# DH-Ng/TacEx

Hardware: AMD Instinct MI355X
Metric: tactile_frames_per_sec (higher is better)
Workload: dtype f32; 1 GPU; 1024 envs x 2 GelSight Mini per GPU = 2048 frames/step/GPU, Taxim RGB 320x240 + FOTS markers (99); BASELINE configs[2] (C3); envs_per_gpu=1024, sensors_per_env=2, markers=True, sensors=group, gather=obs32 u8 (9551872 B/rank, N=1: no collective), arch=gfx950:sramecc+:xnack-

## Files before the change

tacex_amd/csrc/fots_kernels.hip:

```cpp
#include <hip/hip_runtime.h>
#include <math.h>

#include <algorithm>
#include <stdint.h>

#include "tacex_hip.h"
#include "tacex_internal.h"

namespace tacex {

typedef float v4f __attribute__((ext_vector_type(4)));

__global__ __launch_bounds__(1024) void fots_reduce_kernel(const float* __restrict__ z,
                                                          const uint8_t* __restrict__ mask,
                                                          FotsReduce* __restrict__ out, int H, int W) {
  const int e = blockIdx.x;
  const int npix = H * W;
  const float* zz = z + (size_t)e * npix;
  const uint8_t* mm = mask + (size_t)e * npix;
  float zmax = -INFINITY;
  int cnt = 0, sr = 0, sc = 0;
  const int n4 = npix >> 2;
  for (int i = threadIdx.x; i < n4; i += blockDim.x) {
    v4f v = reinterpret_cast<const v4f*>(zz)[i];
    uchar4 m = reinterpret_cast<const uchar4*>(mm)[i];
    zmax = fmaxf(zmax, fmaxf(fmaxf(v[0], v[1]), fmaxf(v[2], v[3])));
    const int p = i << 2;
    const int row = p / W, col = p - row * W;
    const int c = (m.x != 0) + (m.y != 0) + (m.z != 0) + (m.w != 0);
    cnt += c;
    sr += c * row;
    sc += (m.x != 0) * col + (m.y != 0) * (col + 1) + (m.z != 0) * (col + 2) + (m.w != 0) * (col + 3);
  }
#pragma unroll
  for (int o = 32; o > 0; o >>= 1) {
    zmax = fmaxf(zmax, __shfl_xor(zmax, o, 64));
    cnt += __shfl_xor(cnt, o, 64);
    sr += __shfl_xor(sr, o, 64);
    sc += __shfl_xor(sc, o, 64);
  }
  __shared__ float s_z[16];
  __shared__ int s_c[16], s_r[16], s_k[16];
  const int wid = threadIdx.x >> 6;
  if ((threadIdx.x & 63) == 0) { s_z[wid] = zmax; s_c[wid] = cnt; s_r[wid] = sr; s_k[wid] = sc; }
  __syncthreads();
  if (threadIdx.x == 0) {
    const int nw = blockDim.x >> 6;
    for (int w = 1; w < nw; ++w) { zmax = fmaxf(zmax, s_z[w]); cnt += s_c[w]; sr += s_r[w]; sc += s_k[w]; }
    out[e].zmax = zmax; out[e].count = cnt; out[e].sum_row = sr; out[e].sum_col = sc;
  }
}

__global__ __launch_bounds__(64) void fots_combine_kernel(const FotsReduce* __restrict__ part, int n, FotsReduce* __restrict__ out) {
  const int e = blockIdx.x;
  const FotsReduce* p = part + (size_t)e * n;
  float zmax = -INFINITY;
  int cnt = 0, sr = 0, sc = 0;
  for (int i = threadIdx.x; i < n; i += 64) {
    const FotsReduce r = p[i];
    zmax = fmaxf(zmax, r.zmax); cnt += r.count; sr += r.sum_row; sc += r.sum_col;
  }
#pragma unroll
  for (int o = 32; o > 0; o >>= 1) {
    zmax = fmaxf(zmax, __shfl_xor(zmax, o, 64));
    cnt += __shfl_xor(cnt, o, 64);
    sr += __shfl_xor(sr, o, 64);
    sc += __shfl_xor(sc, o, 64);
  }
  if (threadIdx.x == 0) { out[e].zmax = zmax; out[e].count = cnt; out[e].sum_row = sr; out[e].sum_col = sc; }
}

struct FotsArgs {
  const float* z; const uint8_t* mask; const float* indent; const float* theta;
  float* traj; float* markers; const FotsReduce* red;
  const int* mx; const int* my;
  int B, H, W, nrow, ncol;
  int compact;
  double lamb0, lamb1, lamb2;
  float mm2pix, shear_max, theta_max_rad_f;
};

__device__ __forceinline__ int centre_px(float t, float mm2pix, float half) {
  float prod = t * mm2pix;
  asm volatile("" : "+v"(prod));
  return (int)(prod + half);
}

__global__ __launch_bounds__(128) void fots_marker_kernel(FotsArgs a) {
  const int e = blockIdx.x;
  const int M = a.nrow * a.ncol;
  const int tid = threadIdx.x;
  __shared__ float s_gmax;
  __shared__ int s_ncontact;
  __shared__ int s_cy[128], s_cx[128];
  __shared__ double s_ch[128];
  __shared__ int s_flag[128];

  float g = -INFINITY;
  for (int i = tid; i < a.B; i += blockDim.x) g = fmaxf(g, a.red[i].zmax);
#pragma unroll
  for (int o = 32; o > 0; o >>= 1) g = fmaxf(g, __shfl_xor(g, o, 64));
  __shared__ float s_g2[2];
  if ((tid & 63) == 0) s_g2[tid >> 6] = g;
  __syncthreads();
  if (tid == 0) s_gmax = fmaxf(s_g2[0], s_g2[1]);
  __syncthreads();
  const float gmax = s_gmax;
  const FotsReduce red = a.red[e];
  const size_t fo = (size_t)e * a.H * a.W;
  float* out_init = a.markers + (size_t)e * 2 * M * 2;
  float* out_cur = out_init + (size_t)M * 2;
  float* tr = a.traj + (size_t)e * 8;
  const bool in_contact = a.indent[e] > 0.0f;

  const bool active = tid < M;
  int j = 0, i = 0, px = 0, py = 0;
  if (active) { j = tid / a.ncol; i = tid - j * a.ncol; px = a.mx[tid]; py = a.my[tid]; }
  if (active) { out_init[tid * 2 + 0] = (float)px; out_init[tid * 2 + 1] = (float)py; }

  if (!in_contact) {
    if (active) { out_cur[tid * 2 + 0] = (float)px; out_cur[tid * 2 + 1] = (float)py; }
    if (tid == 0) { tr[0] = 0.0f; tr[7] = 0.0f; }
    return;
  }

  bool hit = false;
  float hval = 0.0f;
  if (active && py >= 0 && py < a.H && px >= 0 && px < a.W) {
    const size_t pi = a.compact ? (size_t)e * M + tid : fo + (size_t)py * a.W + px;
    if (a.mask[pi] == 1) {
      hit = true;
      const float dz = gmax - a.z[pi];
      const float dmin = gmax - red.zmax;
      hval = (dz - dmin) / 10.0f;
    }
  }
  s_flag[tid] = hit ? 1 : 0;
  __syncthreads();
  if (hit) {
    const int key = i * a.nrow + j;
    int rank = 0;
    for (int m2 = 0; m2 < M; ++m2) {
      if (s_flag[m2]) {
        const int j2 = m2 / a.ncol, i2 = m2 - j2 * a.ncol;
        rank += (i2 * a.nrow + j2) < key;
      }
    }
    s_cy[rank] = py; s_cx[rank] = px; s_ch[rank] = (double)hval;
  }
  if (tid == 0) {
    int n = 0;
    for (int m2 = 0; m2 < M; ++m2) n += s_flag[m2];
    s_ncontact = n;
  }
  __syncthreads();
  const int nc = s_ncontact;

  float t0x, t0y, t0t, tlx, tly, tlt;
  int tlen;
  {
    const float mean_r = (float)((double)red.sum_row / (double)red.count);
    const float mean_c = (float)((double)red.sum_col / (double)red.count);
    const float cy = (mean_r - (float)(a.H / 2.0)) / a.mm2pix;
    const float cx = (mean_c - (float)(a.W / 2.0)) / a.mm2pix;
    const float th = a.theta[e];
    tlen = (int)tr[0];
    if (tlen == 0) { t0x = cx; t0y = cy; t0t = th; } else { t0x = tr[1]; t0y = tr[2]; t0t = tr[3]; }
    tlx = cx; tly = cy; tlt = th;
    tlen += 1;
  }
  __syncthreads();
  if (tid == 0) {
    tr[0] = (float)tlen; tr[1] = t0x; tr[2] = t0y; tr[3] = t0t; tr[4] = tlx; tr[5] = tly; tr[6] = tlt;
    tr[7] = (float)nc;
  }
  if (!active) return;

  if (nc == 0) {
    out_cur[tid * 2 + 0] = (float)px; out_cur[tid * 2 + 1] = (float)py;
    return;
  }

  double dx = 0.0, dy = 0.0;
  for (int c = 0; c < nc; ++c) {
    const double ox = (double)(px - s_cx[c]), oy = (double)(py - s_cy[c]);
    const double gg = exp(-a.lamb0 * (ox * ox + oy * oy));
    dx += s_ch[c] * ox * gg;
    dy += s_ch[c] * oy * gg;
  }
  double nx = (double)px + dx, ny = (double)py + dy;

  if (tlen >= 2) {
    const float half_w = (float)(a.W / 2.0), half_h = (float)(a.H / 2.0);
    const int scx = centre_px(t0x, a.mm2pix, half_w);
    const int scy = centre_px(t0y, a.mm2pix, half_h);
    int shx = (int)((tlx - t0x) * a.mm2pix);
    int shy = (int)((tly - t0y) * a.mm2pix);
    const int smax = (int)a.shear_max;
    shx = shx < -smax ? -smax : (shx > smax ? smax : shx);
    shy = shy < -smax ? -smax : (shy > smax ? smax : shy);
    {
      const double ox = (double)(px - scx), oy = (double)(py - scy);
      const double gg = exp(-a.lamb1 * (ox * ox + oy * oy));
      nx += (double)shx * gg;
      ny += (double)shy * gg;
    }
    float theta = tlt - t0t;
    theta = fminf(fmaxf(theta, -a.theta_max_rad_f), a.theta_max_rad_f);
    const int tcx = centre_px(tlx, a.mm2pix, half_w);
    const int tcy = centre_px(tly, a.mm2pix, half_h);
    const double c1 = (double)cosf(theta - 1.0f);
    const double s1 = (double)sinf(theta);
    const double ox = (double)(px - tcx), oy = (double)(py - tcy);
    const double gg = exp(-a.lamb2 * (ox * ox + oy * oy));
    nx += (ox * c1 - oy * s1) * gg;
    ny += (ox * s1 + oy * c1) * gg;
  }
  out_cur[tid * 2 + 0] = (float)nx;
  out_cur[tid * 2 + 1] = (float)ny;
}


struct MarkerImgArgs {
  const float* markers;
  const uint8_t* patches;
  const float* rgb;
  uint8_t* img;
  uint8_t* overlay;
  int B, M, H, W, SR, S, patch_w;
  int band_rows, nbands;
};
constexpr int kMkPad = 12, kMkPatch = 12;

__global__ __launch_bounds__(256) void fots_marker_image_kernel(MarkerImgArgs a) {
  extern __shared__ __attribute__((aligned(16))) uint8_t canvas[];
  const int e = blockIdx.x / a.nbands, band = blockIdx.x - e * a.nbands;
  const int CW = a.W + 2 * kMkPad, CH = a.H + 2 * kMkPad;
  const int y0 = band * a.band_rows, y1 = min(CH, y0 + a.band_rows);
  const int tid = threadIdx.x;
  for (int i = tid * 4; i < (y1 - y0) * CW; i += 256 * 4) *reinterpret_cast<uint32_t*>(canvas + i) = 0xffffffffu;
  __syncthreads();
  const float* cur = a.markers + ((size_t)e * 2 + 1) * a.M * 2;
  for (int m = 0; m < a.M; ++m) {
    const double u = ((double)cur[m * 2 + 0] + 0.5) + 12.0, v = ((double)cur[m * 2 + 1] + 0.5) + 12.0;
    const double fu = floor(u), fv = floor(v);
    const int pu = (int)floor((u - fu) * a.SR), pv = (int)floor((v - fv) * a.SR);
    const int cu = (int)fu - 6, cv = (int)fv - 6;
    const bool ok = u == u && v == v && fabs(u) < 1e9 && fabs(v) < 1e9 && cu >= 0 && cu < CW - 12 && cv >= 0 && cv < CH - 12;
    if (ok && cv + kMkPatch > y0 && cv < y1 && tid < kMkPatch * kMkPatch) {
      const int dy = tid / kMkPatch, dx = tid - dy * kMkPatch, yy = cv + dy;
      if (yy >= y0 && yy < y1)
        canvas[(yy - y0) * CW + cu + dx] =
            a.patches[((((size_t)pu * a.SR + pv) * a.S + a.patch_w) * kMkPatch + dy) * kMkPatch + dx];
    }
    __syncthreads();
  }
  const int r0 = max(y0, kMkPad), r1 = min(y1, a.H + kMkPad);
  for (int i = tid; i < (r1 - r0) * a.W; i += 256) {
    const int ry = i / a.W, x = i - ry * a.W;
    const uint8_t mv = canvas[(r0 + ry - y0) * CW + kMkPad + x];
    const size_t p = ((size_t)e * a.H + (r0 + ry - kMkPad)) * a.W + x;
    if (a.img) a.img[p] = mv;
    if (a.overlay) {
      const double f = (double)mv / 255.0;
#pragma unroll
      for (int ch = 0; ch < 3; ++ch) a.overlay[p * 3 + ch] = (uint8_t)(int)((double)(a.rgb[p * 3 + ch] * 255.0f) * f);
    }
  }
}

}

using namespace tacex;

struct tacex_fots_ctx {
  int device = 0;
  int H = 0, W = 0, nrow = 0, ncol = 0;
  int* mx_dev = nullptr;
  int* my_dev = nullptr;
  double lamb[3];
  float mm2pix, shear_max, theta_max_deg;
};

extern "C" {

int tacex_fots_create(int device_id, const tacex_fots_params* p, tacex_fots_ctx** out) {
  if (!p || !out || !p->marker_x || !p->marker_y) { set_error("tacex_fots_create: null argument"); return 2; }
  const int M = p->num_markers_row * p->num_markers_col;
  if (M <= 0 || M > 128) { set_error("tacex_fots_create: %d markers unsupported (1..128)", M); return 2; }
  if (p->width % 4 != 0) { set_error("tacex_fots_create: image width %d must be a multiple of 4", p->width); return 2; }
  hipError_t e = hipSetDevice(device_id);
  if (e != hipSuccess) return fail_hip(e, "hipSetDevice");
  auto* c = new tacex_fots_ctx();
  c->device = device_id; c->H = p->height; c->W = p->width; c->nrow = p->num_markers_row; c->ncol = p->num_markers_col;
  for (int k = 0; k < 3; ++k) c->lamb[k] = p->lamb[k];
  c->mm2pix = p->mm2pix; c->shear_max = p->shear_max; c->theta_max_deg = p->theta_max_deg;
  if ((e = hipMalloc((void**)&c->mx_dev, M * sizeof(int))) != hipSuccess ||
      (e = hipMalloc((void**)&c->my_dev, M * sizeof(int))) != hipSuccess ||
      (e = hipMemcpy(c->mx_dev, p->marker_x, M * sizeof(int), hipMemcpyHostToDevice)) != hipSuccess ||
      (e = hipMemcpy(c->my_dev, p->marker_y, M * sizeof(int), hipMemcpyHostToDevice)) != hipSuccess) {
    tacex_fots_destroy(c);
    return fail_hip(e, "tacex_fots_create: table upload");
  }
  *out = c;
  return 0;
}

void tacex_fots_destroy(tacex_fots_ctx* c) {
  if (!c) return;
  (void)hipSetDevice(c->device);
  if (c->mx_dev) (void)hipFree(c->mx_dev);
  if (c->my_dev) (void)hipFree(c->my_dev);
  delete c;
}

size_t tacex_fots_state_bytes(int num_envs) { return num_envs > 0 ? (size_t)num_envs * 8 * sizeof(float) : 0; }
size_t tacex_fots_workspace_bytes(int num_envs) { return num_envs > 0 ? (size_t)num_envs * sizeof(FotsReduce) : 0; }

static int fots_markers_impl(tacex_fots_ctx* c, const float* z, const uint8_t* mask, const float* indent, const float* theta,
                             float* traj_state, float* markers, void* ws, const FotsReduce* part, int npart, int B, void* stream, int compact = 0);

int tacex_fots_markers(tacex_fots_ctx* c, const float* z, const uint8_t* mask, const float* indent,
                       const float* theta, float* traj_state, float* markers, void* ws, int B, void* stream) {
  if (!c || !z || !mask || !indent || !theta || !traj_state || !markers || !ws) {
    set_error("tacex_fots_markers: null argument");
    return 2;
  }
  if (B <= 0) return 0;
  return fots_markers_impl(c, z, mask, indent, theta, traj_state, markers, ws, nullptr, 0, B, stream);
}

int tacex_fots_markers_partials(tacex_fots_ctx* c, const float* z, const uint8_t* mask, const float* indent,
                                const float* theta, float* traj_state, float* markers, void* ws, const void* partials,
                                int partials_per_env, int B, void* stream) {
  if (!c || !z || !mask || !indent || !theta || !traj_state || !markers || !ws || !partials || partials_per_env < 1) {
    set_error("tacex_fots_markers_partials: null argument");
    return 2;
  }
  if (B <= 0) return 0;
  return fots_markers_impl(c, z, mask, indent, theta, traj_state, markers, ws, static_cast<const FotsReduce*>(partials),
                           partials_per_env, B, stream);
}

int tacex_fots_markers_compact(tacex_fots_ctx* c, const float* z_pix, const uint8_t* mask_pix, const float* indent,
                               const float* theta, float* traj_state, float* markers, void* ws, const void* partials,
                               int partials_per_env, int B, void* stream) {
  if (!c || !z_pix || !mask_pix || !indent || !theta || !traj_state || !markers || !ws || !partials || partials_per_env < 1) {
    set_error("tacex_fots_markers_compact: null argument");
    return 2;
  }
  if (B <= 0) return 0;
  return fots_markers_impl(c, z_pix, mask_pix, indent, theta, traj_state, markers, ws, static_cast<const FotsReduce*>(partials),
                           partials_per_env, B, stream, 1);
}

static int fots_markers_impl(tacex_fots_ctx* c, const float* z, const uint8_t* mask, const float* indent, const float* theta,
                             float* traj_state, float* markers, void* ws, const FotsReduce* part, int npart, int B, void* stream, int compact) {
  hipStream_t st = (hipStream_t)stream;
  FotsReduce* red = static_cast<FotsReduce*>(ws);
  if (part) hipLaunchKernelGGL(fots_combine_kernel, dim3(B), dim3(64), 0, st, part, npart, red);
  else hipLaunchKernelGGL(fots_reduce_kernel, dim3(B), dim3(1024), 0, st, z, mask, red, c->H, c->W);
  FotsArgs a{};
  a.compact = compact;
  a.z = z; a.mask = mask; a.indent = indent; a.theta = theta; a.traj = traj_state; a.markers = markers; a.red = red;
  a.mx = c->mx_dev; a.my = c->my_dev; a.B = B; a.H = c->H; a.W = c->W; a.nrow = c->nrow; a.ncol = c->ncol;
  a.lamb0 = c->lamb[0]; a.lamb1 = c->lamb[1]; a.lamb2 = c->lamb[2];
  a.mm2pix = c->mm2pix; a.shear_max = c->shear_max;
  a.theta_max_rad_f = (float)(c->theta_max_deg / 180.0 * 3.14159265358979323846);
  hipLaunchKernelGGL(fots_marker_kernel, dim3(B), dim3(128), 0, st, a);
  hipError_t e = hipGetLastError();
  if (e != hipSuccess) return fail_hip(e, "fots kernels");
  return 0;
}

int tacex_fots_marker_image(const float* markers, const uint8_t* patches, int super_res, int size_slots, int patch_w,
                            const float* rgb, uint8_t* img, uint8_t* overlay, int B, int M, int H, int W, void* stream) {
  if (!markers || !patches || (!img && !overlay)) { set_error("tacex_fots_marker_image: null argument"); return 2; }
  if (overlay && !rgb) { set_error("tacex_fots_marker_image: the overlay needs the RGB frame"); return 2; }
  if (super_res < 1 || size_slots < 1 || patch_w < 0 || patch_w >= size_slots) {
    set_error("tacex_fots_marker_image: patch table index %d outside [0, %d)", patch_w, size_slots);
    return 2;
  }
  if (W % 4 != 0 || H <= 0 || W <= 0 || M < 0) { set_error("tacex_fots_marker_image: need W %% 4 == 0, H > 0"); return 2; }
  if (B <= 0) return 0;
  MarkerImgArgs a{};
  a.markers = markers; a.patches = patches; a.rgb = rgb; a.img = img; a.overlay = overlay;
  a.B = B; a.M = M; a.H = H; a.W = W; a.SR = super_res; a.S = size_slots; a.patch_w = patch_w;
  const int CW = W + 2 * kMkPad, CH = H + 2 * kMkPad;
  const size_t budget = 96 * 1024;
  a.band_rows = (int)std::min<size_t>((size_t)CH, budget / CW);
  if (a.band_rows < 2 * kMkPatch) { set_error("tacex_fots_marker_image: image too wide (%d)", W); return 2; }
  a.nbands = (CH + a.band_rows - 1) / a.band_rows;
  const size_t lds = (size_t)a.band_rows * CW;
  auto kern = fots_marker_image_kernel;
  static size_t granted[64] = {};
  if (hipError_t e = ensure_dynamic_lds(reinterpret_cast<const void*>(kern), lds, granted); e != hipSuccess)
    return fail_hip(e, "hipFuncSetAttribute(fots_marker_image_kernel)");
  hipLaunchKernelGGL(kern, dim3(B * a.nbands), dim3(256), lds, (hipStream_t)stream, a);
  hipError_t e = hipGetLastError();
  return e == hipSuccess ? 0 : fail_hip(e, "fots_marker_image_kernel");
}

}
```

tacex_amd/csrc/taxim_device.h:

```cpp
#pragma once
#include <hip/hip_runtime.h>
#include <stdint.h>

#include <type_traits>

#include "tacex_internal.h"
#include "wave_ops.h"

namespace tacex {

typedef float v2f __attribute__((ext_vector_type(2)));
typedef float v4f __attribute__((ext_vector_type(4)));

template <int I, int N, typename F>
__device__ __forceinline__ void static_for(F&& f) {
  if constexpr (I < N) {
    f(std::integral_constant<int, I>{});
    static_for<I + 1, N>(f);
  }
}

__device__ __forceinline__ float fmin_raw(float a, float b) {
  float r;
  asm("v_min_f32 %0, %1, %2" : "=v"(r) : "v"(a), "v"(b));
// ... 83 lines not shown
__device__ __forceinline__ void shade_bins(const ShadeArgs& a, float ztop, float zbot, float zlef, float zrig, int& im,
                                           int& id) {
  const float dzdx = (ztop - zbot) * a.gsy;
  const float dzdy = (zlef - zrig) * a.gsx;
  const float t = __builtin_amdgcn_sqrtf(fmaf(dzdx, dzdx, dzdy * dzdy));
  const float mag = atan_pos(t);
  const float dir = t != 0.0f ? atan2_fast(dzdx, dzdy) : 0.0f;
  im = min((int)(mag * a.inv_x_binr), a.nb - 1);
  id = min((int)((dir + 3.14159274101257324f) * a.inv_y_binr), a.nb - 1);
}

__device__ __forceinline__ int shade_dir_bin(const ShadeArgs& a, float dzdx, float dzdy, float t2) {
  const float dir = !(t2 < 1.17549435e-38f) ? atan2_fast(dzdx, dzdy) : 0.0f;
  return min((int)((dir + 3.14159274101257324f) * a.inv_y_binr), a.nb - 1);
}
__device__ __forceinline__ int shade_mag_bin(const ShadeArgs& a, float t2) {
  return min((int)(atan_pos(__builtin_amdgcn_sqrtf(t2)) * a.inv_x_binr), a.nb - 1);
}

__device__ __forceinline__ void shade_poly(const ShadeArgs& a, int im, int id, float X, float Y, float out[3]) {
  const v4f* __restrict__ pc =
      reinterpret_cast<const v4f*>(reinterpret_cast<const char*>(a.poly) + (unsigned)(im * a.nb + id) * 96u);
  const v4f c0 = pc[0], c1 = pc[1], c2 = pc[2], c3 = pc[3], c4 = pc[4];
  const float f0 = X * X, f1 = Y * Y, f2 = X * Y;
  out[0] = fmaf(f0, c0.x, fmaf(f1, c0.y, fmaf(f2, c0.z, fmaf(X, c0.w, fmaf(Y, c1.x, c1.y)))));
  out[1] = fmaf(f0, c1.z, fmaf(f1, c1.w, fmaf(f2, c2.x, fmaf(X, c2.y, fmaf(Y, c2.z, c2.w)))));
  out[2] = fmaf(f0, c3.x, fmaf(f1, c3.y, fmaf(f2, c3.z, fmaf(X, c3.w, fmaf(Y, c4.x, c4.y)))));
}

__device__ __forceinline__ void shade_pixel_core(const ShadeArgs& a, float ztop, float zbot, float zlef, float zrig,
                                                 int x, int y, float out[3], int& im_out, int& id_out) {
  const unsigned p = (unsigned)y * (unsigned)a.W + (unsigned)x;
  int im, id;
  shade_bins(a, ztop, zbot, zlef, zrig, im, id);
  float c[3];
  shade_poly(a, im, id, a.fx[(unsigned)x], a.fy[(unsigned)y], c);
  const float* __restrict__ bg = reinterpret_cast<const float*>(reinterpret_cast<const char*>(a.bg) + p * 12u);
  out[0] = __builtin_amdgcn_fmed3f(c[0] + bg[0], 0.0f, 1.0f);
  out[1] = __builtin_amdgcn_fmed3f(c[1] + bg[1], 0.0f, 1.0f);
  out[2] = __builtin_amdgcn_fmed3f(c[2] + bg[2], 0.0f, 1.0f);
  im_out = im;
  id_out = id;
}

__device__ __forceinline__ void shade_pixel_rgb(const ShadeArgs& a, float ztop, float zbot, float zlef, float zrig, int x,
                                                int y, float out[3]) {
  int im, id;
  shade_pixel_core(a, ztop, zbot, zlef, zrig, x, y, out, im, id);
}

__device__ __forceinline__ void shade_strip4_rgb(const ShadeArgs& a, const float zn[4][4], int x, int y, float out[12]) {
  const unsigned p = (unsigned)y * (unsigned)a.W + (unsigned)x;
  const v4f X4 = *reinterpret_cast<const v4f*>(a.fx + (unsigned)x);
  const float Y = a.fy[(unsigned)y];
  const v4f* __restrict__ bgp = reinterpret_cast<const v4f*>(reinterpret_cast<const char*>(a.bg) + p * 12u);
  const v4f b0 = bgp[0], b1 = bgp[1], b2 = bgp[2];
  const float bg[12] = {b0.x, b0.y, b0.z, b0.w, b1.x, b1.y, b1.z, b1.w, b2.x, b2.y, b2.z, b2.w};
#pragma unroll
  for (int i = 0; i < 4; ++i) {
    int im, id;
    shade_bins(a, zn[i][0], zn[i][1], zn[i][2], zn[i][3], im, id);
    float c[3];
    shade_poly(a, im, id, X4[i], Y, c);
#pragma unroll
    for (int ch = 0; ch < 3; ++ch) out[3 * i + ch] = __builtin_amdgcn_fmed3f(c[ch] + bg[3 * i + ch], 0.0f, 1.0f);
  }
}

__device__ __forceinline__ void shade_pixel(const ShadeArgs& a, float ztop, float zbot, float zlef, float zrig, int x,
                                            int y, int b) {
  float c[3];
  int im, id;
  shade_pixel_core(a, ztop, zbot, zlef, zrig, x, y, c, im, id);
  const size_t p = (size_t)y * a.W + x;
  float* __restrict__ o = a.rgb + ((size_t)b * a.H * a.W + p) * 3;
  o[0] = c[0]; o[1] = c[1]; o[2] = c[2];
  if (a.idx_out) {
    uint8_t* io = a.idx_out + ((size_t)b * a.H * a.W + p) * 2;
    io[0] = (uint8_t)im;
    io[1] = (uint8_t)id;
  }
}

template <bool U8, typename G>
__device__ __forceinline__ void obs_finish_cell(void* __restrict__ obs_v, const ObsTables& T, G&& gather) {
  const int oh = T.oh, ow = T.ow;
  const int cell = blockIdx.x * blockDim.x + threadIdx.x;
  if (cell >= oh * ow) return;
  const int b = blockIdx.y;
  const int oy = cell / ow, ox = cell - oy * ow;
  float a0 = 0.0f, a1 = 0.0f, a2 = 0.0f;
  gather(b, oy, ox, a0, a1, a2);
  const float nrm = T.xsum[ox] * T.ysum[oy];
  const size_t oi = ((size_t)b * (oh * ow) + cell) * 3;
  if constexpr (U8) {
    uint8_t* o = static_cast<uint8_t*>(obs_v) + oi;
    o[0] = (uint8_t)(a0 / nrm * 255.0f + 0.5f); o[1] = (uint8_t)(a1 / nrm * 255.0f + 0.5f); o[2] = (uint8_t)(a2 / nrm * 255.0f + 0.5f);
  } else {
    float* o = static_cast<float*>(obs_v) + oi;
    o[0] = a0 / nrm; o[1] = a1 / nrm; o[2] = a2 / nrm;
  }
}
template <typename K, typename... A>
inline hipError_t launch_obs_finish(bool u8, K kern_u8, K kern_f32, const ObsTables& t, int B, hipStream_t st, A... args) {
  const dim3 grid((t.oh * t.ow + 255) / 256, B);
  hipLaunchKernelGGL(u8 ? kern_u8 : kern_f32, grid, dim3(256), 0, st, args...);
  return hipGetLastError();
}

}
```

tacex_amd/csrc/taxim_stream.hip:

```cpp
#include <hip/hip_runtime.h>
#include <stdint.h>
#include <stdlib.h>

#include <type_traits>
#include <vector>

#include "tacex_internal.h"
#include "taxim_device.h"

namespace tacex {

constexpr int kStreamPx = 3;
constexpr int kStreamWaves = 4;
constexpr int kStreamObsActive = 3;

struct StreamArgs {
  const float* zin;
  const float* hm;
  const float* gel;
  const float* shift_a;
  const float* shift_b;
  const float* pdepth;
  const float* taps[kStreamMaxLevels];
  ShadeArgs sh;
// ... 902 lines not shown
    if (do_obs) {
      obs_flush(OA[0], cur_o0);
      obs_flush(OA[1], cur_o0 + 1);
      obs_flush(OA[2], cur_o0 + 2);
    }
  }
  if (do_fots) {
    f_zmax = wave_scan_max_lane63(f_zmax);
    int f_sc = 0;
#pragma unroll
    for (int i = 0; i < PX; ++i) f_sc += f_cpx[i] * xg[i];
    f_sc = wave_scan_add_lane63(f_sc);
    if (lane == 63) {
      FotsReduce r;
      r.zmax = f_zmax; r.count = f_cnt; r.sum_row = f_sr; r.sum_col = f_sc;
      a.fots_part[(size_t)frame * a.fots_stride + rem] = r;
    }
    if (rem == 0) {
      FotsReduce id;
      id.zmax = -INFINITY; id.count = 0; id.sum_row = 0; id.sum_col = 0;
      for (int s2 = per_frame + lane; s2 < a.fots_stride; s2 += 64) a.fots_part[(size_t)frame * a.fots_stride + s2] = id;
    }
  }
}

__global__ __launch_bounds__(256) void stream_flat_image_kernel(ShadeArgs sh, float* __restrict__ out) {
  const int x = blockIdx.x * blockDim.x + threadIdx.x, y = blockIdx.y;
  if (x >= sh.W) return;
  const int code = shade_dir_bin(sh, 0.0f, 0.0f, 0.0f);
  const StreamRec r = stream_rec_load(sh.poly + (size_t)code * 24);
  float p0, p1, p2;
  stream_poly(sh.fx[x], sh.fy[y], r, p0, p1, p2);
  const float* bg = sh.bg + ((size_t)y * sh.W + x) * 3;
  float* o = out + ((size_t)y * sh.W + x) * 3;
  o[0] = __builtin_amdgcn_fmed3f(p0 + bg[0], 0.0f, 1.0f);
  o[1] = __builtin_amdgcn_fmed3f(p1 + bg[1], 0.0f, 1.0f);
  o[2] = __builtin_amdgcn_fmed3f(p2 + bg[2], 0.0f, 1.0f);
}

__global__ __launch_bounds__(1024) void stream_order_kernel(const int* __restrict__ rows_ext, int n_items, int per_frame, int nseg,
                                                            int seg_rows, int H, int reach, int* __restrict__ order) {
  constexpr int kKeys = 1024;
  __shared__ int hist[kKeys], start[kKeys];
  for (int k = threadIdx.x; k < kKeys; k += blockDim.x) hist[k] = 0;
  __syncthreads();
  auto key_of = [&](int item) {
    const int frame = item / per_frame, seg = (item - frame * per_frame) % nseg;
    const int r0 = seg * seg_rows, r1 = min(H, r0 + seg_rows);
    const int lo = rows_ext[4 * frame], hi = rows_ext[4 * frame + 1];
    if ((r0 - reach > hi) || (r1 + reach < lo)) return 0;
    const int pad = 4;
    const int c = min(r1 - 1, hi + pad) - max(r0, lo - pad) + 1;
    return min(kKeys - 1, 1 + max(c, 0));
  };
  for (int i = threadIdx.x; i < n_items; i += blockDim.x) atomicAdd(&hist[key_of(i)], 1);
  __syncthreads();
  if (threadIdx.x == 0) {
    int acc = 0;
    for (int k = min(kKeys - 1, seg_rows + 9); k >= 0; --k) { start[k] = acc; acc += hist[k]; }
  }
  __syncthreads();
  for (int i = threadIdx.x; i < n_items; i += blockDim.x) order[atomicAdd(&start[key_of(i)], 1)] = i;
}

template <bool U8>
__global__ __launch_bounds__(256) void obs_finish_stream_kernel(const float* __restrict__ part, void* __restrict__ obs_v, ObsTables T,
                                                               const int* __restrict__ strip_q0, const int* __restrict__ strip_nq,
                                                               const int* __restrict__ seg_oa, const int* __restrict__ seg_ob,
                                                               int nstrips, int nseg, int nrows, int ncols) {
  obs_finish_cell<U8>(obs_v, T, [&](int b, int oy, int ox, float& a0, float& a1, float& a2) {
    for (int s = 0; s < nstrips; ++s) {
      const int qi = ox - strip_q0[s];
      if (qi < 0 || qi >= strip_nq[s]) continue;
      for (int g = 0; g < nseg; ++g) {
        if (oy < seg_oa[g] || oy > seg_ob[g]) continue;
        const size_t blk = ((size_t)b * nstrips + s) * nseg + g;
        const float* pp = part + blk * ((size_t)nrows * ncols * 3) + ((size_t)(oy - seg_oa[g]) * ncols + qi) * 3;
        a0 += pp[0]; a1 += pp[1]; a2 += pp[2];
      }
    }
  });
}

template <int ROLE, bool ST, int... KS>
constexpr StreamCfg<ROLE, KS...> stream_cfg(FusedSet<ST, KS...>) { return {}; }

template <typename C>
static bool stream_geometry_t(int W, int* nstrips, int* strip_w) {
  int ns = (W + C::VW - 1) / C::VW;
  int sw = (((W + ns - 1) / ns) + 3) & ~3;
  if (sw > C::VW) { ++ns; sw = (((W + ns - 1) / ns) + 3) & ~3; }
  *nstrips = ns;
  *strip_w = sw;
  return sw <= C::VW;
}

static bool stream_split() {
  static const int v = getenv("TACEX_STREAM_SPLIT") ? atoi(getenv("TACEX_STREAM_SPLIT")) : 0;
  return v != 0;
}

bool stream_supported(int n_fused, int k0, int H, int W) {
  static const int en = getenv("TACEX_TAIL_STREAM") ? atoi(getenv("TACEX_TAIL_STREAM")) : 1;
  return en != 0 && with_stream_set(n_fused, k0, false, [](auto) { return true; }) && H >= 16 && W >= 16 && W % 4 == 0;
}

bool stream_geometry(int n_fused, int k0, int W, int* nstrips, int* strip_w, int* lv_nstrips, int* lv_strip_w) {
  return with_stream_set(n_fused, k0, false, [&](auto s) {
    if (stream_split())
      return stream_geometry_t<StreamCfg<kStreamShade>>(W, nstrips, strip_w) &&
             stream_geometry_t<decltype(stream_cfg<kStreamLevels>(s))>(W, lv_nstrips, lv_strip_w);
    const bool ok = stream_geometry_t<decltype(stream_cfg<kStreamFused>(s))>(W, nstrips, strip_w);
    *lv_nstrips = *nstrips; *lv_strip_w = *strip_w;
    return ok;
  });
}

int stream_segments(int B, int nstrips, int H, int warm, int per_simd) {
  static const int forced = getenv("TACEX_STREAM_SEGS") ? atoi(getenv("TACEX_STREAM_SEGS")) : 0;
  int nseg = forced > 0 ? forced : (1024 * per_simd + B * nstrips - 1) / (B * nstrips);
  if (nseg < 1) nseg = 1;
  if (nseg > kStreamMaxSeg) nseg = kStreamMaxSeg;
  const int min_rows = forced > 0 ? 24 : (3 * warm > 24 ? 3 * warm : 24);
  while (nseg > 1 && (H / nseg < min_rows || H - (nseg - 1) * ((H + nseg - 1) / nseg) < 4)) --nseg;
  return nseg;
}
int stream_waves_per_simd(int n_fused, int k0) {
  return with_stream_set(n_fused, k0, 2, [](auto s) { return decltype(stream_cfg<kStreamFused>(s))::min_waves(); });
}
static int stream_sum_r(int n_fused, int k0) {
  return with_stream_set(n_fused, k0, 0, [](auto s) { return decltype(stream_cfg<kStreamFused>(s))::sum_r(); });
}
int stream_warm_rows(int n_fused, int k0, bool levels_kernel) {
  const int sum_r = stream_sum_r(n_fused, k0);
  if (!stream_split()) return 2 * sum_r + 2;
  return levels_kernel ? 2 * sum_r : 2;
}

template <bool GZ, int ROLE, int... KS>
static hipError_t launch_stream_k(const StreamArgs& a, hipStream_t st) {
  using C = StreamCfg<ROLE, KS...>;
  const int waves = a.B * a.nstrips * a.nseg;
  const int nwg = (waves + kStreamWaves - 1) / kStreamWaves;
  const dim3 grid(nwg);
  static const size_t lds_pad = getenv("TACEX_STREAM_LDS_PAD") ? (size_t)atoi(getenv("TACEX_STREAM_LDS_PAD")) : 0;
  const size_t lds = C::lds_bytes() + lds_pad;
  auto kern = taxim_stream_kernel<GZ, ROLE, C::min_waves(), KS...>;
  static size_t granted[64] = {};
  if (hipError_t e = ensure_dynamic_lds(reinterpret_cast<const void*>(kern), lds, granted); e != hipSuccess) return e;
  hipLaunchKernelGGL(kern, grid, dim3(64 * kStreamWaves), lds, st, a);
  return hipGetLastError();
}

template <int ROLE, bool ST, int... KS>
static hipError_t launch_stream(FusedSet<ST, KS...>, const StreamArgs& a, bool gel_zero, hipStream_t st) {
  return gel_zero ? launch_stream_k<true, ROLE, KS...>(a, st) : launch_stream_k<false, ROLE, KS...>(a, st);
}

hipError_t run_stream_flat_image(const ShadeParams* sp, int H, int W, hipStream_t st) {
  if (!sp->flat_rgb_dev) return hipErrorInvalidValue;
  hipLaunchKernelGGL(stream_flat_image_kernel, dim3((W + 255) / 256, H), dim3(256), 0, st, make_shade_args(*sp, 1, H, W), sp->flat_rgb_dev);
  return hipGetLastError();
}

static bool stream_sorted() {
  static const int sorted = getenv("TACEX_STREAM_ORDER") ? atoi(getenv("TACEX_STREAM_ORDER")) : 1;
// ... 7 lines not shown
  return hipGetLastError();
}

hipError_t run_stream_order(const LevelDesc* lv, int n_levels, int n_fused, const StreamPlan& plan, int B, int H, const int* rows_ext, int ext_grow,
                            int* order_buf, hipStream_t st, bool* launched) {
  *launched = false;
  if (stream_split() || !stream_sorted() || !order_buf || !lv[0].gel_zero || !rows_ext) return hipSuccess;
  const hipError_t e = launch_stream_order(stream_sum_r(n_fused, lv[n_levels - n_fused].kw), rows_ext, ext_grow, B, plan.nstrips, plan.nseg,
                                           plan.seg_rows, H, order_buf, st);
  *launched = e == hipSuccess;
  return e;
}

bool stream_tail_range_aware(const LevelDesc* lv) {
#ifdef TACEX_STREAM_HM_ALWAYS
  return false;
#else
  return lv[0].gel_zero;
#endif
}

hipError_t run_stream_tail(const LevelDesc* lv, int n_levels, int n_fused, const float* zin, const float* hm, const float* gel,
                           const float* sa, const float* sb, const float* pd, const ShadeParams* sp, float* rgb, float* z_last,
                           int B, int H, int W, float contact_scale, const StreamPlan& plan, float* obs_part,
                           FotsReduce* fots_part, int fots_stride, float* pix_z, uint8_t* pix_m, hipStream_t st,
                           const int* rows_ext, int ext_grow, int* order_buf, bool order_done) {
  const bool sorted = stream_sorted();
  StreamArgs a{};
  a.rows_ext = lv[0].gel_zero ? rows_ext : nullptr; a.ext_grow = ext_grow;
  a.zin = zin; a.hm = hm; a.gel = lv[0].gel_zero ? nullptr : gel; a.shift_a = sa; a.shift_b = sb; a.pdepth = pd;
  a.H = H; a.W = W; a.B = B; a.contact_scale = contact_scale;
  for (int i = 0; i < n_fused; ++i) a.taps[i] = lv[n_levels - n_fused + i].taps_w_dev;
  a.sh = make_shade_args(*sp, B, H, W);
  a.sh.rgb = rgb;
#ifndef TACEX_STREAM_NO_TRIM
  a.flat_rgb = sp->flat_rgb_dev;
#endif
  {
    const double t1 = tan((double)sp->x_binr) * (1.0 - 2e-5);
    a.mag0_t2 = (float)(t1 * t1);
  }
  a.rows = static_cast<const int*>(plan.rows); a.mk_vec = plan.mk_vec ? 1 : 0;
  StreamArgs sh = a;
  sh.nstrips = plan.nstrips; sh.strip_w = plan.strip_w; sh.nseg = plan.nseg; sh.seg_rows = plan.seg_rows;
  if (obs_part && plan.obs_ready) {
    sh.obs_part = obs_part;
    sh.obs_kxp = plan.obs_kxp;
    sh.obs_xlo = plan.obs.xlo; sh.obs_xcnt = plan.obs.xcnt; sh.obs_wx = plan.obs.wx; sh.obs_kx = plan.obs.kx;
    sh.obs_strip_q0 = plan.obs_strip_q0; sh.obs_strip_nq = plan.obs_strip_nq;
    sh.obs_seg_oa = plan.obs_seg_oa; sh.obs_seg_ob = plan.obs_seg_ob;
    sh.obs_nrows = plan.obs_nrows; sh.obs_ncols = plan.obs_ncols;
  }
  StreamArgs lvl = a;
  lvl.nstrips = plan.lv_nstrips; lvl.strip_w = plan.lv_strip_w; lvl.nseg = plan.lv_nseg; lvl.seg_rows = plan.lv_seg_rows;
  StreamArgs& f = stream_split() ? lvl : sh;
  f.fots_part = fots_part; f.fots_stride = fots_stride;
  if (pix_z && pix_m && plan.mk_x) {
    f.pix_z = pix_z; f.pix_m = pix_m; f.n_markers = plan.n_markers;
    f.mk_x = plan.mk_x; f.mk_id = plan.mk_id;
  }
  const int k0 = lv[n_levels - n_fused].kw;
  const bool gz = lv[0].gel_zero;
  if (!stream_split()) {
    if (order_done) {
      sh.order = order_buf;
    } else if (sorted && order_buf && gz && rows_ext) {
      if (hipError_t e = launch_stream_order(stream_sum_r(n_fused, k0), rows_ext, ext_grow, B, sh.nstrips, sh.nseg, sh.seg_rows, H, order_buf, st);
          e != hipSuccess)
        return e;
      sh.order = order_buf;
    }
    return with_stream_set(n_fused, k0, hipErrorInvalidValue, [&](auto s) { return launch_stream<kStreamFused>(s, sh, gz, st); });
  }
  if (!z_last) return hipErrorInvalidValue;
  lvl.z_out = z_last;
  if (hipError_t e = with_stream_set(n_fused, k0, hipErrorInvalidValue, [&](auto s) { return launch_stream<kStreamLevels>(s, lvl, gz, st); });
      e != hipSuccess)
    return e;
  sh.zin = z_last;
  return launch_stream<kStreamShade>(FusedSet<true>{}, sh, true, st);
}

hipError_t run_obs_finish_stream(const float* part, void* obs, bool u8, const StreamPlan& plan, int B, hipStream_t st) {
  return launch_obs_finish(u8, obs_finish_stream_kernel<true>, obs_finish_stream_kernel<false>, plan.obs, B, st, part, obs, plan.obs,
                           plan.obs_strip_q0, plan.obs_strip_nq, plan.obs_seg_oa, plan.obs_seg_ob, plan.nstrips, plan.nseg, plan.obs_nrows,
                           plan.obs_ncols);
}

#ifdef TACEX_STREAM_PROBE_DEEP
template __global__ void taxim_stream_kernel<true, kStreamFused, 2, 17, 9, 5, 3, 5>(StreamArgs);
template __global__ void taxim_stream_kernel<true, kStreamFused, 2, 15, 9, 5, 9>(StreamArgs);
static_assert(StreamCfg<kStreamFused, 17, 9, 5, 3, 5>::lds_bytes() > 80 * 1024, "deep variant: one workgroup per CU");
#endif

int stream_obs_lds_floats() { return kStreamObsLdsFloats; }
int stream_obs_max_cols() { return kStreamObsMaxCols; }

}
```

tacex_amd/csrc/wave_ops.h:

```cpp
#pragma once
#include <hip/hip_runtime.h>

namespace tacex {

__device__ __forceinline__ float wave_min(float v) {
#pragma unroll
  for (int o = 32; o > 0; o >>= 1) v = fminf(v, __shfl_xor(v, o, 64));
  return v;
}
__device__ __forceinline__ float wave_max(float v) {
#pragma unroll
  for (int o = 32; o > 0; o >>= 1) v = fmaxf(v, __shfl_xor(v, o, 64));
  return v;
}

#define TACEX_DPP_SCAN(v, IDENT, OP, T_AS_INT, INT_AS_T)                                                              \
  do {                                                                                                                \
    v = OP(v, INT_AS_T(__builtin_amdgcn_update_dpp(T_AS_INT(IDENT), T_AS_INT(v), 0x111, 0xf, 0xf, false)));           \
    v = OP(v, INT_AS_T(__builtin_amdgcn_update_dpp(T_AS_INT(IDENT), T_AS_INT(v), 0x112, 0xf, 0xf, false)));           \
    v = OP(v, INT_AS_T(__builtin_amdgcn_update_dpp(T_AS_INT(IDENT), T_AS_INT(v), 0x114, 0xf, 0xf, false)));           \
    v = OP(v, INT_AS_T(__builtin_amdgcn_update_dpp(T_AS_INT(IDENT), T_AS_INT(v), 0x118, 0xf, 0xf, false)));           \
    v = OP(v, INT_AS_T(__builtin_amdgcn_update_dpp(T_AS_INT(IDENT), T_AS_INT(v), 0x142, 0xa, 0xf, false)));           \
    v = OP(v, INT_AS_T(__builtin_amdgcn_update_dpp(T_AS_INT(IDENT), T_AS_INT(v), 0x143, 0xc, 0xf, false)));           \
  } while (0)
__device__ __forceinline__ int dpp_id_int(int x) { return x; }
__device__ __forceinline__ int dpp_add_int(int a, int b) { return a + b; }
__device__ __forceinline__ int wave_scan_add_lane63(int v) {
  TACEX_DPP_SCAN(v, 0, dpp_add_int, dpp_id_int, dpp_id_int);
  return v;
}
__device__ __forceinline__ float wave_scan_min_lane63(float v) {
  TACEX_DPP_SCAN(v, INFINITY, fminf, __float_as_int, __int_as_float);
  return v;
}
__device__ __forceinline__ float wave_scan_max_lane63(float v) {
  TACEX_DPP_SCAN(v, -INFINITY, fmaxf, __float_as_int, __int_as_float);
  return v;
}

}
```

Measured before the change: 760,900 frames/s.

## Precompute FOTS pair weights, ballot-rank contacts, vectorise obs finish stores

The FOTS marker kernel now reads dilation weights from a pairwise table precomputed at create time instead of calling exp per contact. It iterates markers in column-major order so contact ranks come from a wave ballot and mbcnt rather than an O(M) shared-memory scan. The global zmax is read from a packed float array with vector loads instead of a strided struct. A separate obs-finish kernel handles four output cells per thread with vectorised partial loads and packed u8 stores. The costs are an M*M double table and extra memory reads in place of arithmetic. Env vars can switch both paths off.

```diff
diff --git a/tacex_amd/csrc/fots_kernels.hip b/tacex_amd/csrc/fots_kernels.hip
--- a/tacex_amd/csrc/fots_kernels.hip
+++ b/tacex_amd/csrc/fots_kernels.hip
@@ -3,9 +3,11 @@
 
 #include <algorithm>
 #include <stdint.h>
+#include <stdlib.h>
 
 #include "tacex_hip.h"
 #include "tacex_internal.h"
+#include "wave_ops.h"
 
 namespace tacex {
 
@@ -13,7 +15,8 @@
 
 __global__ __launch_bounds__(1024) void fots_reduce_kernel(const float* __restrict__ z,
                                                           const uint8_t* __restrict__ mask,
-                                                          FotsReduce* __restrict__ out, int H, int W) {
+                                                          FotsReduce* __restrict__ out, float* __restrict__ zmax_out, int H,
+                                                          int W) {
   const int e = blockIdx.x;
   const int npix = H * W;
   const float* zz = z + (size_t)e * npix;
@@ -48,10 +51,12 @@
     const int nw = blockDim.x >> 6;
     for (int w = 1; w < nw; ++w) { zmax = fmaxf(zmax, s_z[w]); cnt += s_c[w]; sr += s_r[w]; sc += s_k[w]; }
     out[e].zmax = zmax; out[e].count = cnt; out[e].sum_row = sr; out[e].sum_col = sc;
-  }
-}
-
-__global__ __launch_bounds__(64) void fots_combine_kernel(const FotsReduce* __restrict__ part, int n, FotsReduce* __restrict__ out) {
+    if (zmax_out) zmax_out[e] = zmax;
+  }
+}
+
+__global__ __launch_bounds__(64) void fots_combine_kernel(const FotsReduce* __restrict__ part, int n, FotsReduce* __restrict__ out,
+                                                          float* __restrict__ zmax_out) {
   const int e = blockIdx.x;
   const FotsReduce* p = part + (size_t)e * n;
   float zmax = -INFINITY;
@@ -67,7 +72,10 @@
     sr += __shfl_xor(sr, o, 64);
     sc += __shfl_xor(sc, o, 64);
   }
-  if (threadIdx.x == 0) { out[e].zmax = zmax; out[e].count = cnt; out[e].sum_row = sr; out[e].sum_col = sc; }
+  if (threadIdx.x == 0) {
+    out[e].zmax = zmax; out[e].count = cnt; out[e].sum_row = sr; out[e].sum_col = sc;
+    if (zmax_out) zmax_out[e] = zmax;
+  }
 }
 
 struct FotsArgs {
@@ -78,7 +86,35 @@
   int compact;
   double lamb0, lamb1, lamb2;
   float mm2pix, shear_max, theta_max_rad_f;
+  const double* pair;
+  const float* zmax;
 };
+
+__device__ __forceinline__ double fots_dilate_weight(double lamb0, double ox, double oy) {
+  return exp(-lamb0 * (ox * ox + oy * oy));
+}
+
+__device__ __forceinline__ int fots_marker_at(int v, int nrow, int ncol, int& j, int& i) {
+  i = v / nrow;
+  j = v - i * nrow;
+  return j * ncol + i;
+}
+
+__global__ __launch_bounds__(128) void fots_pair_table_kernel(const int* __restrict__ mx, const int* __restrict__ my, int nrow, int ncol,
+                                                             double lamb0, double* __restrict__ pair) {
+  const int M = nrow * ncol, vc = blockIdx.x, v = threadIdx.x;
+  if (v >= M) return;
+  int j, i;
+  const int mc = fots_marker_at(vc, nrow, ncol, j, i), m = fots_marker_at(v, nrow, ncol, j, i);
+  const double ox = (double)(mx[m] - mx[mc]), oy = (double)(my[m] - my[mc]);
+  pair[(size_t)vc * M + v] = fots_dilate_weight(lamb0, ox, oy);
+}
+
+__device__ __forceinline__ int fots_wave_rank(bool flag, int* total) {
+  const unsigned long long b = __ballot(flag);
+  *total = __popcll(b);
+  return wave_mbcnt(b);
+}
 
 __device__ __forceinline__ int centre_px(float t, float mm2pix, float half) {
   float prod = t * mm2pix;
@@ -86,18 +122,40 @@
   return (int)(prod + half);
 }
 
+template <bool FAST>
 __global__ __launch_bounds__(128) void fots_marker_kernel(FotsArgs a) {
   const int e = blockIdx.x;
   const int M = a.nrow * a.ncol;
   const int tid = threadIdx.x;
   __shared__ float s_gmax;
   __shared__ int s_ncontact;
-  __shared__ int s_cy[128], s_cx[128];
+  __shared__ int s_cy[128], s_cx[128], s_cv[128];
   __shared__ double s_ch[128];
   __shared__ int s_flag[128];
+  __shared__ int s_wtot[2];
 
   float g = -INFINITY;
-  for (int i = tid; i < a.B; i += blockDim.x) g = fmaxf(g, a.red[i].zmax);
+  if constexpr (FAST) {
+    constexpr int kTrips = 4;
+    for (int base = 0; base < a.B; base += 128 * 4 * kTrips) {
+      v4f v[kTrips];
+#pragma unroll
+      for (int k = 0; k < kTrips; ++k) {
+        const int i0 = base + (k * 128 + tid) * 4;
+        v[k] = v4f{-INFINITY, -INFINITY, -INFINITY, -INFINITY};
+        if (i0 + 3 < a.B) {
+          v[k] = *reinterpret_cast<const v4f*>(a.zmax + i0);
+        } else {
+          for (int q = 0; q < 3; ++q)
+            if (i0 + q < a.B) v[k][q] = a.zmax[i0 + q];
+        }
+      }
+#pragma unroll
+      for (int k = 0; k < kTrips; ++k) g = fmaxf(g, fmaxf(fmaxf(v[k][0], v[k][1]), fmaxf(v[k][2], v[k][3])));
+    }
+  } else {
+    for (int i = tid; i < a.B; i += blockDim.x) g = fmaxf(g, a.red[i].zmax);
+  }
 #pragma unroll
   for (int o = 32; o > 0; o >>= 1) g = fmaxf(g, __shfl_xor(g, o, 64));
   __shared__ float s_g2[2];
@@ -114,12 +172,15 @@
   const bool in_contact = a.indent[e] > 0.0f;
 
   const bool active = tid < M;
-  int j = 0, i = 0, px = 0, py = 0;
-  if (active) { j = tid / a.ncol; i = tid - j * a.ncol; px = a.mx[tid]; py = a.my[tid]; }
-  if (active) { out_init[tid * 2 + 0] = (float)px; out_init[tid * 2 + 1] = (float)py; }
+  int j = 0, i = 0, px = 0, py = 0, m = tid;
+  if (active) {
+    if constexpr (FAST) { m = fots_marker_at(tid, a.nrow, a.ncol, j, i); } else { j = tid / a.ncol; i = tid - j * a.ncol; }
+    px = a.mx[m]; py = a.my[m];
+  }
+  if (active) { out_init[m * 2 + 0] = (float)px; out_init[m * 2 + 1] = (float)py; }
 
   if (!in_contact) {
-    if (active) { out_cur[tid * 2 + 0] = (float)px; out_cur[tid * 2 + 1] = (float)py; }
+    if (active) { out_cur[m * 2 + 0] = (float)px; out_cur[m * 2 + 1] = (float)py; }
     if (tid == 0) { tr[0] = 0.0f; tr[7] = 0.0f; }
     return;
   }
@@ -127,7 +188,7 @@
   bool hit = false;
   float hval = 0.0f;
   if (active && py >= 0 && py < a.H && px >= 0 && px < a.W) {
-    const size_t pi = a.compact ? (size_t)e * M + tid : fo + (size_t)py * a.W + px;
+    const size_t pi = a.compact ? (size_t)e * M + m : fo + (size_t)py * a.W + px;
     if (a.mask[pi] == 1) {
       hit = true;
       const float dz = gmax - a.z[pi];
@@ -135,26 +196,39 @@
       hval = (dz - dmin) / 10.0f;
     }
   }
-  s_flag[tid] = hit ? 1 : 0;
-  __syncthreads();
-  if (hit) {
-    const int key = i * a.nrow + j;
-    int rank = 0;
-    for (int m2 = 0; m2 < M; ++m2) {
-      if (s_flag[m2]) {
-        const int j2 = m2 / a.ncol, i2 = m2 - j2 * a.ncol;
-        rank += (i2 * a.nrow + j2) < key;
+  int nc;
+  if constexpr (FAST) {
+    int total;
+    const int below = fots_wave_rank(hit, &total);
+    if ((tid & 63) == 0) s_wtot[tid >> 6] = total;
+    __syncthreads();
+    nc = s_wtot[0] + s_wtot[1];
+    if (hit) {
+      const int rank = below + (tid >= 64 ? s_wtot[0] : 0);
+      s_cy[rank] = py; s_cx[rank] = px; s_cv[rank] = tid; s_ch[rank] = (double)hval;
+    }
+  } else {
+    s_flag[tid] = hit ? 1 : 0;
+    __syncthreads();
+    if (hit) {
+      const int key = i * a.nrow + j;
+      int rank = 0;
+      for (int m2 = 0; m2 < M; ++m2) {
+        if (s_flag[m2]) {
+          const int j2 = m2 / a.ncol, i2 = m2 - j2 * a.ncol;
+          rank += (i2 * a.nrow + j2) < key;
+        }
       }
-    }
-    s_cy[rank] = py; s_cx[rank] = px; s_ch[rank] = (double)hval;
-  }
-  if (tid == 0) {
-    int n = 0;
-    for (int m2 = 0; m2 < M; ++m2) n += s_flag[m2];
-    s_ncontact = n;
-  }
-  __syncthreads();
-  const int nc = s_ncontact;
+      s_cy[rank] = py; s_cx[rank] = px; s_ch[rank] = (double)hval;
+    }
+    if (tid == 0) {
+      int n = 0;
+      for (int m2 = 0; m2 < M; ++m2) n += s_flag[m2];
+      s_ncontact = n;
+    }
+    __syncthreads();
+    nc = s_ncontact;
+  }
 
   float t0x, t0y, t0t, tlx, tly, tlt;
   int tlen;
@@ -177,14 +251,16 @@
   if (!active) return;
 
   if (nc == 0) {
-    out_cur[tid * 2 + 0] = (float)px; out_cur[tid * 2 + 1] = (float)py;
+    out_cur[m * 2 + 0] = (float)px; out_cur[m * 2 + 1] = (float)py;
     return;
   }
 
   double dx = 0.0, dy = 0.0;
   for (int c = 0; c < nc; ++c) {
     const double ox = (double)(px - s_cx[c]), oy = (double)(py - s_cy[c]);
-    const double gg = exp(-a.lamb0 * (ox * ox + oy * oy));
+    double gg;
+    if constexpr (FAST) gg = a.pair[s_cv[c] * M + tid];
+    else gg = fots_dilate_weight(a.lamb0, ox, oy);
     dx += s_ch[c] * ox * gg;
     dy += s_ch[c] * oy * gg;
   }
@@ -216,8 +292,8 @@
     nx += (ox * c1 - oy * s1) * gg;
     ny += (ox * s1 + oy * c1) * gg;
   }
-  out_cur[tid * 2 + 0] = (float)nx;
-  out_cur[tid * 2 + 1] = (float)ny;
+  out_cur[m * 2 + 0] = (float)nx;
+  out_cur[m * 2 + 1] = (float)ny;
 }
 
 
@@ -278,6 +354,9 @@
   int H = 0, W = 0, nrow = 0, ncol = 0;
   int* mx_dev = nullptr;
   int* my_dev = nullptr;
+  double* pair_dev = nullptr;
+  float* zmax_dev = nullptr;
+  int zmax_cap = 0;
   double lamb[3];
   float mm2pix, shear_max, theta_max_deg;
 };
@@ -302,6 +381,14 @@
     tacex_fots_destroy(c);
     return fail_hip(e, "tacex_fots_create: table upload");
   }
+  if ((e = hipMalloc((void**)&c->pair_dev, (size_t)M * M * sizeof(double))) == hipSuccess) {
+    hipLaunchKernelGGL(fots_pair_table_kernel, dim3(M), dim3(128), 0, nullptr, c->mx_dev, c->my_dev, c->nrow, c->ncol, c->lamb[0], c->pair_dev);
+    if ((e = hipGetLastError()) == hipSuccess) e = hipDeviceSynchronize();
+  }
+  if (e != hipSuccess) {
+    tacex_fots_destroy(c);
+    return fail_hip(e, "tacex_fots_create: pair table");
+  }
   *out = c;
   return 0;
 }
@@ -311,6 +398,8 @@
   (void)hipSetDevice(c->device);
   if (c->mx_dev) (void)hipFree(c->mx_dev);
   if (c->my_dev) (void)hipFree(c->my_dev);
+  if (c->pair_dev) (void)hipFree(c->pair_dev);
+  if (c->zmax_dev) (void)hipFree(c->zmax_dev);
   delete c;
 }
 
@@ -358,16 +447,26 @@
                              float* traj_state, float* markers, void* ws, const FotsReduce* part, int npart, int B, void* stream, int compact) {
   hipStream_t st = (hipStream_t)stream;
   FotsReduce* red = static_cast<FotsReduce*>(ws);
-  if (part) hipLaunchKernelGGL(fots_combine_kernel, dim3(B), dim3(64), 0, st, part, npart, red);
-  else hipLaunchKernelGGL(fots_reduce_kernel, dim3(B), dim3(1024), 0, st, z, mask, red, c->H, c->W);
+  static const bool fast = !(getenv("TACEX_FOTS_PAIR_TABLE") && atoi(getenv("TACEX_FOTS_PAIR_TABLE")) == 0);
+  if (fast && B > c->zmax_cap) {
+    if (c->zmax_dev) (void)hipFree(c->zmax_dev);
+    c->zmax_dev = nullptr; c->zmax_cap = 0;
+    const int cap = (B + 3) & ~3;
+    if (hipError_t em = hipMalloc((void**)&c->zmax_dev, (size_t)cap * sizeof(float)); em != hipSuccess) return fail_hip(em, "hipMalloc(fots maxima)");
+    c->zmax_cap = cap;
+  }
+  float* zmax = fast ? c->zmax_dev : nullptr;
+  if (part) hipLaunchKernelGGL(fots_combine_kernel, dim3(B), dim3(64), 0, st, part, npart, red, zmax);
+  else hipLaunchKernelGGL(fots_reduce_kernel, dim3(B), dim3(1024), 0, st, z, mask, red, zmax, c->H, c->W);
   FotsArgs a{};
+  a.pair = c->pair_dev; a.zmax = zmax;
   a.compact = compact;
   a.z = z; a.mask = mask; a.indent = indent; a.theta = theta; a.traj = traj_state; a.markers = markers; a.red = red;
   a.mx = c->mx_dev; a.my = c->my_dev; a.B = B; a.H = c->H; a.W = c->W; a.nrow = c->nrow; a.ncol = c->ncol;
   a.lamb0 = c->lamb[0]; a.lamb1 = c->lamb[1]; a.lamb2 = c->lamb[2];
   a.mm2pix = c->mm2pix; a.shear_max = c->shear_max;
   a.theta_max_rad_f = (float)(c->theta_max_deg / 180.0 * 3.14159265358979323846);
-  hipLaunchKernelGGL(fots_marker_kernel, dim3(B), dim3(128), 0, st, a);
+  hipLaunchKernelGGL(fast ? fots_marker_kernel<true> : fots_marker_kernel<false>, dim3(B), dim3(128), 0, st, a);
   hipError_t e = hipGetLastError();
   if (e != hipSuccess) return fail_hip(e, "fots kernels");
   return 0;
diff --git a/tacex_amd/csrc/taxim_device.h b/tacex_amd/csrc/taxim_device.h
--- a/tacex_amd/csrc/taxim_device.h
+++ b/tacex_amd/csrc/taxim_device.h
@@ -189,6 +189,18 @@
   }
 }
 
+__device__ __forceinline__ uint8_t obs_norm_u8(float a, float nrm) { return (uint8_t)(a / nrm * 255.0f + 0.5f); }
+template <bool U8>
+__device__ __forceinline__ void obs_store_cell(void* __restrict__ obs_v, size_t cell, float a0, float a1, float a2, float nrm) {
+  if constexpr (U8) {
+    uint8_t* o = static_cast<uint8_t*>(obs_v) + cell * 3;
+    o[0] = obs_norm_u8(a0, nrm); o[1] = obs_norm_u8(a1, nrm); o[2] = obs_norm_u8(a2, nrm);
+  } else {
+    float* o = static_cast<float*>(obs_v) + cell * 3;
+    o[0] = a0 / nrm; o[1] = a1 / nrm; o[2] = a2 / nrm;
+  }
+}
+
 template <bool U8, typename G>
 __device__ __forceinline__ void obs_finish_cell(void* __restrict__ obs_v, const ObsTables& T, G&& gather) {
   const int oh = T.oh, ow = T.ow;
@@ -198,15 +210,7 @@
   const int oy = cell / ow, ox = cell - oy * ow;
   float a0 = 0.0f, a1 = 0.0f, a2 = 0.0f;
   gather(b, oy, ox, a0, a1, a2);
-  const float nrm = T.xsum[ox] * T.ysum[oy];
-  const size_t oi = ((size_t)b * (oh * ow) + cell) * 3;
-  if constexpr (U8) {
-    uint8_t* o = static_cast<uint8_t*>(obs_v) + oi;
-    o[0] = (uint8_t)(a0 / nrm * 255.0f + 0.5f); o[1] = (uint8_t)(a1 / nrm * 255.0f + 0.5f); o[2] = (uint8_t)(a2 / nrm * 255.0f + 0.5f);
-  } else {
-    float* o = static_cast<float*>(obs_v) + oi;
-    o[0] = a0 / nrm; o[1] = a1 / nrm; o[2] = a2 / nrm;
-  }
+  obs_store_cell<U8>(obs_v, (size_t)b * (oh * ow) + cell, a0, a1, a2, T.xsum[ox] * T.ysum[oy]);
 }
 template <typename K, typename... A>
 inline hipError_t launch_obs_finish(bool u8, K kern_u8, K kern_f32, const ObsTables& t, int B, hipStream_t st, A... args) {
diff --git a/tacex_amd/csrc/taxim_stream.hip b/tacex_amd/csrc/taxim_stream.hip
--- a/tacex_amd/csrc/taxim_stream.hip
+++ b/tacex_amd/csrc/taxim_stream.hip
@@ -1008,6 +1008,81 @@
   });
 }
 
+template <bool U8>
+__global__ __launch_bounds__(256) void obs_finish_stream4_kernel(const float* __restrict__ part, void* __restrict__ obs_v, ObsTables T,
+                                                                const int* __restrict__ strip_q0, const int* __restrict__ strip_nq,
+                                                                const int* __restrict__ seg_oa, const int* __restrict__ seg_ob,
+                                                                int nstrips, int nseg, int nrows, int ncols) {
+  const int oh = T.oh, ow = T.ow, gpr = (ow + 3) >> 2;
+  const int grp = blockIdx.x * blockDim.x + threadIdx.x;
+  if (grp >= oh * gpr) return;
+  const int b = blockIdx.y;
+  const int oy = grp / gpr, ox0 = (grp - oy * gpr) << 2;
+  const int nx = min(4, ow - ox0);
+  float acc[12];
+#pragma unroll
+  for (int k = 0; k < 12; ++k) acc[k] = 0.0f;
+  for (int s = 0; s < nstrips; ++s) {
+    const int qi0 = ox0 - strip_q0[s], nq = strip_nq[s];
+    if (qi0 + nx <= 0 || qi0 >= nq) continue;
+    const bool whole = nx == 4 && qi0 >= 0 && qi0 + 4 <= nq;
+    for (int g = 0; g < nseg; ++g) {
+      if (oy < seg_oa[g] || oy > seg_ob[g]) continue;
+      const size_t blk = ((size_t)b * nstrips + s) * nseg + g;
+      const float* pp = part + blk * ((size_t)nrows * ncols * 3) + ((ptrdiff_t)(oy - seg_oa[g]) * ncols + qi0) * 3;
+      if (whole) {
+        if ((reinterpret_cast<uintptr_t>(pp) & 15u) == 0) {
+          const v4f* p4 = reinterpret_cast<const v4f*>(pp);
+          const v4f v0 = p4[0], v1 = p4[1], v2 = p4[2];
+#pragma unroll
+          for (int k = 0; k < 4; ++k) { acc[k] += v0[k]; acc[4 + k] += v1[k]; acc[8 + k] += v2[k]; }
+        } else {
+          float v[12];
+#pragma unroll
+          for (int k = 0; k < 12; ++k) v[k] = pp[k];
+#pragma unroll
+          for (int k = 0; k < 12; ++k) acc[k] += v[k];
+        }
+      } else {
+#pragma unroll
+        for (int c = 0; c < 4; ++c) {
+          if (c >= nx || qi0 + c < 0 || qi0 + c >= nq) continue;
+          acc[3 * c] += pp[3 * c]; acc[3 * c + 1] += pp[3 * c + 1]; acc[3 * c + 2] += pp[3 * c + 2];
+        }
+      }
+    }
+  }
+  const float ys = T.ysum[oy];
+  const size_t cell0 = (size_t)b * (oh * ow) + (size_t)oy * ow + ox0;
+  if (nx == 4 && (cell0 & 3) == 0) {
+    if constexpr (U8) {
+      uint32_t w[3];
+#pragma unroll
+      for (int k = 0; k < 3; ++k) {
+        uint32_t v = 0;
+#pragma unroll
+        for (int q = 0; q < 4; ++q) {
+          const int i = 4 * k + q;
+          v |= (uint32_t)obs_norm_u8(acc[i], T.xsum[ox0 + i / 3] * ys) << (8 * q);
+        }
+        w[k] = v;
+      }
+      uint32_t* o = reinterpret_cast<uint32_t*>(static_cast<uint8_t*>(obs_v) + cell0 * 3);
+      o[0] = w[0]; o[1] = w[1]; o[2] = w[2];
+    } else {
+      v4f w[3];
+#pragma unroll
+      for (int i = 0; i < 12; ++i) w[i >> 2][i & 3] = acc[i] / (T.xsum[ox0 + i / 3] * ys);
+      v4f* o = reinterpret_cast<v4f*>(static_cast<float*>(obs_v) + cell0 * 3);
+      o[0] = w[0]; o[1] = w[1]; o[2] = w[2];
+    }
+  } else {
+#pragma unroll
+    for (int c = 0; c < 4; ++c)
+      if (c < nx) obs_store_cell<U8>(obs_v, cell0 + c, acc[3 * c], acc[3 * c + 1], acc[3 * c + 2], T.xsum[ox0 + c] * ys);
+  }
+}
+
 template <int ROLE, bool ST, int... KS>
 constexpr StreamCfg<ROLE, KS...> stream_cfg(FusedSet<ST, KS...>) { return {}; }
 
@@ -1181,6 +1256,14 @@
 }
 
 hipError_t run_obs_finish_stream(const float* part, void* obs, bool u8, const StreamPlan& plan, int B, hipStream_t st) {
+  static const bool vec = !(getenv("TACEX_OBS_FINISH_VEC") && atoi(getenv("TACEX_OBS_FINISH_VEC")) == 0);
+  if (vec) {
+    const int groups = plan.obs.oh * ((plan.obs.ow + 3) / 4);
+    hipLaunchKernelGGL(u8 ? obs_finish_stream4_kernel<true> : obs_finish_stream4_kernel<false>, dim3((groups + 255) / 256, B), dim3(256), 0, st, part, obs,
+                       plan.obs, plan.obs_strip_q0, plan.obs_strip_nq, plan.obs_seg_oa, plan.obs_seg_ob, plan.nstrips, plan.nseg, plan.obs_nrows,
+                       plan.obs_ncols);
+    return hipGetLastError();
+  }
   return launch_obs_finish(u8, obs_finish_stream_kernel<true>, obs_finish_stream_kernel<false>, plan.obs, B, st, part, obs, plan.obs,
                            plan.obs_strip_q0, plan.obs_strip_nq, plan.obs_seg_oa, plan.obs_seg_ob, plan.nstrips, plan.nseg, plan.obs_nrows,
                            plan.obs_ncols);
diff --git a/tacex_amd/csrc/wave_ops.h b/tacex_amd/csrc/wave_ops.h
--- a/tacex_amd/csrc/wave_ops.h
+++ b/tacex_amd/csrc/wave_ops.h
@@ -12,6 +12,10 @@
 #pragma unroll
   for (int o = 32; o > 0; o >>= 1) v = fmaxf(v, __shfl_xor(v, o, 64));
   return v;
+}
+
+__device__ __forceinline__ int wave_mbcnt(unsigned long long ballot) {
+  return (int)__builtin_amdgcn_mbcnt_hi((unsigned)(ballot >> 32), __builtin_amdgcn_mbcnt_lo((unsigned)ballot, 0u));
 }
 
 #define TACEX_DPP_SCAN(v, IDENT, OP, T_AS_INT, INT_AS_T)                                                              \
```

Result: no change. 765,200 frames/s, median of 5 (+0.6%).
